# Innoptech/OpenFDCM

Hardware: AMD Instinct MI355X
Metric: template matches/sec (DT3 build + DefaultMatch/BatchOptimize search per frame) (higher is better)
Workload: dtype f32

## Files before the change

openfdcm_amd/csrc/fdcm_search.hip:

```cpp
#include <algorithm>
#include <cstdio>
#include <atomic>
#include <chrono>
#include <cstring>
#include <numeric>
#include <thread>

#include "fdcm_internal.h"
#include "fdcm_score.h"

namespace fdcm {

struct SearchParams {
    const float* vol;
    const float* keys;
    int W, H, m;
    float tx, ty;
    const float* tlines;
    const long long* toffsets;
    const float* tlengths;
    const int* tsorted;
    int T;
    const float* slines;
    const float* s_sorted_len;
    const int* s_sorted_idx;
    int n_s;
    int maxT, maxS, window;
    int optimizer;
    int batch;
    int win;
    int base;
    const long long* cand_offsets;
    const int2* pairs;
    int pairs_stride;
    int bpt;
    const int2* work;
    long long ncand;
    int nblocks;
    int lds_lines;
    const unsigned short* host_bins;
    fdcm_match* records;
    int* flags;
    int* evals;
    unsigned long long* counters;
};

static constexpr int kWavesPerBlock = 4;

struct OptState {
    VolRef V;
    const float* L;
    float* sc;
    int n_t, lane, B, WIN;
    bool batch_rule;
    bool reset_back;
    unsigned H;
    float tx, ty, savx, savy;
    int lim_p, lim_n;
};

template <bool BUF32>
__device__ __forceinline__ void score_range(const OptState& o, int dir, int k_from, int cnt, int dst, bool with_zero) {
    const int h = o.lane >> 5, slot = o.lane & 31;
    const int total = cnt + (with_zero ? 1 : 0);
    for (int s0 = 0; s0 < total; s0 += 32) {
        const int idx = s0 + slot - (with_zero ? 1 : 0);
        const bool act = idx < cnt;
        const int k = idx < 0 ? 0 : k_from + dir * idx;
        const float trx = idx < 0 ? 0.f : (float)k * o.savx, try_ = idx < 0 ? 0.f : (float)k * o.savy;
        const float s = pair_score<BUF32>(o.V, o.L, o.n_t, o.tx + trx, o.ty + try_, o.H, h, act);
        if (act && h == 0) o.sc[idx < 0 ? 2 * o.WIN : dst + idx] = s;
    }
}

template <bool BUF32>
__device__ __forceinline__ void optimise(const OptState& o, float& best, int& best_k, int& n_eval) {
    const int WIN = o.WIN, B = o.B;
    const int h = o.lane >> 5, slot = o.lane & 31;
    const int have_p = min(WIN, o.lim_p >= 1 ? o.lim_p : 0);
    const int have_n = min(WIN, o.lim_n <= -1 ? -o.lim_n : 0);
    if (1 + have_p + have_n <= 32) {
        const int idx = slot - 1;
        const bool is_p = idx >= 0 && idx < have_p, is_n = idx >= have_p && idx < have_p + have_n;
        const bool act = slot == 0 || is_p || is_n;
        const int k = is_p ? 1 + idx : (is_n ? -1 - (idx - have_p) : 0);
        const float trx = slot == 0 ? 0.f : (float)k * o.savx, try_ = slot == 0 ? 0.f : (float)k * o.savy;
        const float s = pair_score<BUF32>(o.V, o.L, o.n_t, o.tx + trx, o.ty + try_, o.H, h, act);
        if (act && h == 0) o.sc[slot == 0 ? 2 * WIN : (is_p ? idx : WIN + (idx - have_p))] = s;
    } else {
        score_range<BUF32>(o, +1, 1, have_p, 0, true);
        score_range<BUF32>(o, -1, -1, have_n, WIN, false);
    }
    const float init = o.sc[2 * WIN];
    n_eval += 1;
    best = init;
    float back = init;
    for (int dir = 1; dir >= -1; dir -= 2) {
        if (dir < 0 && o.reset_back) back = init;
        const int lim = dir > 0 ? o.lim_p : o.lim_n;
        const int off = dir > 0 ? 0 : WIN;
        int win0 = dir;
        int have = dir > 0 ? have_p : have_n;
        for (int k0 = dir; dir > 0 ? k0 <= lim : k0 >= lim; k0 += dir * B) {
            int nb = dir > 0 ? (lim - k0 + 1) : (k0 - lim + 1);
            if (nb > B) nb = B;
            float bmin = 0.f, blast = 0.f;
            int bmin_k = 0;
            for (int c0 = 0; c0 < nb;) {
                int rel = dir > 0 ? (k0 + c0 - win0) : (win0 - (k0 - c0));
                if (rel >= have) {
                    win0 = k0 + dir * c0;
                    const int left = dir > 0 ? (lim - win0 + 1) : (win0 - lim + 1);
                    have = min(WIN, left);
                    score_range<BUF32>(o, dir, win0, have, off, false);
                    rel = 0;
                }
                const int take = min(nb - c0, have - rel);
                for (int e0 = 0; e0 < take; e0 += 64) {
                    const int n = min(64, take - e0);
                    const float s = o.lane < n ? o.sc[off + rel + e0 + o.lane] : f_inf();
                    const bool is_nan = s != s;
                    const unsigned long long nans = __ballot(is_nan);
                    const float mn = wave_min_f(is_nan ? f_inf() : s);
                    const unsigned long long at = __ballot(o.lane < n && !is_nan && s == mn);
                    if (c0 == 0 && e0 == 0 && (nans & 1ull)) {
                        bmin = f_nan(); bmin_k = k0;
                    } else if (at != 0 && ((c0 == 0 && e0 == 0) || mn < bmin)) {
                        bmin = mn; bmin_k = k0 + dir * (c0 + e0 + __ffsll((long long)at) - 1);
                    }
                    blast = __shfl(s, n - 1);
                }
                c0 += take;
            }
            n_eval += nb;
            if (bmin > back) break;
            back = bmin;
            if (bmin < best) { best = bmin; best_k = bmin_k; }
            if (o.batch_rule && bmin < blast) break;
        }
    }
}

__global__ void k_pairs(const SearchParams P) {
    const int gidx = blockIdx.x * blockDim.x + threadIdx.x;
    const int per = P.maxT;
    if (gidx >= P.T * per) return;
    const int t = gidx / per, j = gidx - t * per;
    const long long l0 = P.toffsets[t];
    const int n_t = (int)(P.toffsets[t + 1] - l0);
    int2* out = const_cast<int2*>(P.pairs) + (size_t)t * P.pairs_stride + (size_t)j * P.window;
    if (j >= n_t) {
        for (int wi = 0; wi < P.window; ++wi) out[wi] = make_int2(-1, -1);
        return;
    }
    const int tl_local = P.tsorted[l0 + j];
    const float tlen = P.tlengths[l0 + tl_local];
    const int centre = binary_search_greater(P.s_sorted_len, P.n_s, tlen);
    int rb, re;
    centered_range(centre, P.n_s, P.maxS, rb, re);
    for (int wi = 0; wi < P.window; ++wi) out[wi] = make_int2(tl_local, P.s_sorted_idx[rb + wi]);
}

static constexpr int kWorkBins = 8192;
__device__ __forceinline__ int work_key(int scene_idx) { return scene_idx & (kWorkBins - 1); }
__device__ __forceinline__ int work_rank(int* bins, int key, bool valid, int lane) {
    (void)lane;
    return valid ? atomicAdd(&bins[key], 1) : 0;
}
__device__ __forceinline__ void work_scan(int* bins, int* partial, int tid) {
    constexpr int PER = kWorkBins / 1024;
    int loc[PER], sum = 0;
#pragma unroll
    for (int q = 0; q < PER; ++q) { loc[q] = sum; sum += bins[tid * PER + q]; }
    partial[tid] = sum;
    __syncthreads();
    for (int d = 1; d < 1024; d <<= 1) {
        const int v = tid >= d ? partial[tid - d] : 0;
        __syncthreads();
        partial[tid] += v;
        __syncthreads();
    }
    const int excl = partial[tid] - sum;
#pragma unroll
    for (int q = 0; q < PER; ++q) bins[tid * PER + q] = excl + loc[q];
}

__global__ void __launch_bounds__(1024) k_worklist(const SearchParams P, long long n_slots, int2* __restrict__ work) {
    __shared__ int bins[kWorkBins];
    __shared__ int partial[1024];
    const int tid = threadIdx.x, lane = tid & 63;
    for (int i = tid; i < kWorkBins; i += 1024) bins[i] = 0;
    {
        constexpr int RR = 16;
        int2 pr[RR];
        int rk[RR];
#pragma unroll
        for (int r = 0; r < RR; ++r) {
            const long long i = (long long)r * 1024 + tid;
            pr[r] = i < n_slots ? P.pairs[i] : make_int2(-1, -1);
        }
        __syncthreads();
#pragma unroll
        for (int r = 0; r < RR; ++r) rk[r] = work_rank(bins, work_key(pr[r].y), pr[r].x >= 0, lane);
        __syncthreads();
        work_scan(bins, partial, tid);
        __syncthreads();
#pragma unroll
        for (int r = 0; r < RR; ++r) {
            if (pr[r].x < 0) continue;
            const long long i = (long long)r * 1024 + tid;
            const int t = (int)(i / P.pairs_stride);
            work[bins[work_key(pr[r].y)] + rk[r]] = make_int2(t, (int)(i - (long long)t * P.pairs_stride));
        }
    }
}

static constexpr int kWlSlotsPerBlock = 16 * 1024;
__global__ void __launch_bounds__(1024) k_wl_count(const SearchParams P, long long n_slots, int* __restrict__ ghist) {
    __shared__ int bins[kWorkBins];
    const int tid = threadIdx.x;
    for (int i = tid; i < kWorkBins; i += 1024) bins[i] = 0;
    __syncthreads();
    const long long b0 = (long long)blockIdx.x * kWlSlotsPerBlock;
#pragma unroll
    for (int r = 0; r < 16; ++r) {
        const long long i = b0 + (long long)r * 1024 + tid;
        const int2 pr = i < n_slots ? P.pairs[i] : make_int2(-1, -1);
        if (pr.x >= 0) atomicAdd(&bins[work_key(pr.y)], 1);
    }
    __syncthreads();
    for (int i = tid; i < kWorkBins; i += 1024)
        if (bins[i]) atomicAdd(&ghist[i], bins[i]);
}
__global__ void __launch_bounds__(1024) k_wl_starts(int* __restrict__ ghist, int* __restrict__ cursor) {
    __shared__ int bins[kWorkBins];
    __shared__ int partial[1024];
    const int tid = threadIdx.x;
    for (int i = tid; i < kWorkBins; i += 1024) { bins[i] = ghist[i]; cursor[i] = 0; }
    __syncthreads();
    work_scan(bins, partial, tid);
    __syncthreads();
    for (int i = tid; i < kWorkBins; i += 1024) ghist[i] = bins[i];
}
__global__ void __launch_bounds__(1024) k_wl_scatter(const SearchParams P, long long n_slots, const int* __restrict__ starts,
                                                     int* __restrict__ cursor, int2* __restrict__ work) {
    __shared__ int bins[kWorkBins];
    const int tid = threadIdx.x, lane = tid & 63;
    for (int i = tid; i < kWorkBins; i += 1024) bins[i] = 0;
    __syncthreads();
    const long long b0 = (long long)blockIdx.x * kWlSlotsPerBlock;
    int2 pr[16];
    int rk[16];
#pragma unroll
    for (int r = 0; r < 16; ++r) {
        const long long i = b0 + (long long)r * 1024 + tid;
        pr[r] = i < n_slots ? P.pairs[i] : make_int2(-1, -1);
    }
#pragma unroll
    for (int r = 0; r < 16; ++r) rk[r] = work_rank(bins, work_key(pr[r].y), pr[r].x >= 0, lane);
    __syncthreads();
    for (int i = tid; i < kWorkBins; i += 1024) {
        const int c = bins[i];
        bins[i] = c ? starts[i] + atomicAdd(&cursor[i], c) : 0;
    }
    __syncthreads();
#pragma unroll
    for (int r = 0; r < 16; ++r) {
        if (pr[r].x < 0) continue;
        const long long i = b0 + (long long)r * 1024 + tid;
        const int t = (int)(i / P.pairs_stride);
        work[bins[work_key(pr[r].y)] + rk[r]] = make_int2(t, (int)(i - (long long)t * P.pairs_stride));
    }
}

static constexpr int kSearchWavesPerEU = 4;
template <bool BUF32>
__global__ void __launch_bounds__(64 * kWavesPerBlock, kSearchWavesPerEU) k_search(const SearchParams P) {
    extern __shared__ float lds[];
    const int tid = threadIdx.x, lane = tid & 63, wave = tid >> 6;
    int t, local;
    if (P.work) {
        const long long w = (long long)blockIdx.x * kWavesPerBlock + wave;
        if (w >= P.ncand) return;
        const int2 e = P.work[w >> 1];
        t = e.x;
        local = e.y * 2 + (int)(w & 1);
    } else {
        t = blockIdx.x / P.bpt;
        local = (blockIdx.x - t * P.bpt) * kWavesPerBlock + wave;
    }
    const long long l0 = P.toffsets[t];
    const int n_t = (int)(P.toffsets[t + 1] - l0);
    const int count_t = 2 * min(n_t, P.maxT) * P.window;
    if (local >= count_t) return;
    float* s_keys = lds + (size_t)wave * (P.m + 5 * P.lds_lines + 2 * P.win + 1);
    float* L = s_keys + P.m;
    float* sc = L + 5 * P.lds_lines;
    for (int i = lane; i < P.m; i += 64) s_keys[i] = P.keys[i];
    const long long cand = P.cand_offsets[t] + local;
    const VolRef V = make_volref(P.vol, ivol_slice_floats(P.W, P.H), P.m, BUF32);

    const int flip = local & 1, pair = local >> 1;
    const int2 pr = P.pairs[(size_t)t * P.pairs_stride + pair];
    const int tl_local = pr.x, scene_idx = pr.y;
    float tl[4], sl[4];
#pragma unroll
    for (int c = 0; c < 4; ++c) { tl[c] = P.tlines[(l0 + tl_local) * 4 + c]; sl[c] = P.slines[(size_t)scene_idx * 4 + c]; }
    const float* s_tl = P.tlines + l0 * 4;
    float T1[6], T2[6], T[6];
    align_pair(tl, sl, T1, T2);
#pragma unroll
    for (int c = 0; c < 6; ++c) T[c] = flip ? T2[c] : T1[c];
    float mnx = f_inf(), mny = f_inf(), mxx = -f_inf(), mxy = -f_inf();
    for (int i = lane; i < n_t; i += 64) {
        const float* p = s_tl + 4 * i;
        const float x1 = (T[0] * p[0] + T[1] * p[1]) + T[2], y1 = (T[3] * p[0] + T[4] * p[1]) + T[5];
        const float x2 = (T[0] * p[2] + T[1] * p[3]) + T[2], y2 = (T[3] * p[2] + T[4] * p[3]) + T[5];
        int bin;
        if (P.host_bins) {
            bin = (int)P.host_bins[(size_t)cand * P.lds_lines + i];
        } else {
            const float angle = atanf_glibc((y2 - y1) / (x2 - x1));
            bin = closest_orientation(s_keys, P.m, angle);
        }
        float* d = L + 5 * i;
        d[0] = x1; d[1] = y1; d[2] = x2; d[3] = y2; d[4] = line_slice_word(V, bin);
        mnx = std_min(mnx, std_min(x1, x2)); mxx = std_max(mxx, std_max(x1, x2));
        mny = std_min(mny, std_min(y1, y2)); mxy = std_max(mxy, std_max(y1, y2));
    }
    mnx = wave_min_f(mnx); mny = wave_min_f(mny); mxx = wave_max_f(mxx); mxy = wave_max_f(mxy);

    bool valid = true;
    float ax = sl[2] - sl[0], ay = sl[3] - sl[1];
    {
        const float nrm = sqrtf(ax * ax + ay * ay);
        ax = ax / nrm; ay = ay / nrm;
    }
    if (relatively_equal(f_abs(ax) + f_abs(ay), 0.f)) valid = false;
    float savx = 0.f, savy = 0.f, min_mul = 0.f, max_mul = 0.f;
    if (valid) {
        rasterize_vector(ax, ay, savx, savy);
        minmax_translation(mnx, mny, mxx, mxy, savx, savy, (float)P.W, (float)P.H, P.tx, P.ty, min_mul, max_mul);
        if (!f_isfinite(min_mul) || !f_isfinite(max_mul)) valid = false;
    }
    float best = 0.f;
    int best_k = 0, n_eval = 0;
    if (valid) {
        OptState o;
        o.V = V; o.L = L; o.sc = sc; o.n_t = n_t; o.H = (unsigned)P.H; o.tx = P.tx; o.ty = P.ty;
        o.savx = savx; o.savy = savy; o.lane = lane;
        o.B = P.optimizer == FDCM_BATCH_OPTIMIZE ? P.batch : 1; o.WIN = P.win; o.batch_rule = P.optimizer == FDCM_BATCH_OPTIMIZE;
        o.reset_back = P.optimizer == FDCM_INDULGENT_OPTIMIZE;
        const long long lp = (long long)max_mul, ln = (long long)min_mul;
        o.lim_p = (int)std::min<long long>(std::max<long long>(lp, -(1ll << 30)), 1ll << 30);
        o.lim_n = (int)std::min<long long>(std::max<long long>(ln, -(1ll << 30)), 1ll << 30);
        optimise<BUF32>(o, best, best_k, n_eval);
    }
    if (lane == 0) {
        fdcm_match r;
        r.tmpl_idx = P.base + t;
        r.score = best;
        const float trx = best_k == 0 ? 0.f : (float)best_k * savx, try_ = best_k == 0 ? 0.f : (float)best_k * savy;
        r.transform[0] = T[0]; r.transform[1] = T[1]; r.transform[2] = T[2] + trx;
        r.transform[3] = T[3]; r.transform[4] = T[4]; r.transform[5] = T[5] + try_;
        if (valid) P.records[cand] = r;
        P.flags[cand] = valid ? 1 : 0;
        P.evals[cand] = (int)n_eval;
    }
}

static constexpr int kChunk = 1024;
__global__ void __launch_bounds__(256) k_chunk_counts(const int* __restrict__ flags, const int* __restrict__ evals,
                                                      long long n, int* __restrict__ counts, int* __restrict__ evsums) {
    __shared__ int part[4], epart[4];
    const long long c0 = (long long)blockIdx.x * kChunk;
    int s = 0, e = 0;
    for (int i = threadIdx.x; i < kChunk; i += 256) {
        if (c0 + i < n) { s += flags[c0 + i]; e += evals[c0 + i]; }
    }
    for (int d = 32; d >= 1; d >>= 1) { s += __shfl_xor(s, d); e += __shfl_xor(e, d); }
    if ((threadIdx.x & 63) == 0) { part[threadIdx.x >> 6] = s; epart[threadIdx.x >> 6] = e; }
    __syncthreads();
    if (threadIdx.x == 0) {
        counts[blockIdx.x] = part[0] + part[1] + part[2] + part[3];
        evsums[blockIdx.x] = epart[0] + epart[1] + epart[2] + epart[3];
    }
}
__global__ void __launch_bounds__(1024) k_scatter(const fdcm_match* __restrict__ records, const int* __restrict__ flags,
                                                  long long n, const int* __restrict__ counts,
                                                  const int* __restrict__ evsums, int nchunks,
                                                  fdcm_match* __restrict__ out, unsigned long long* __restrict__ counters,
                                                  fdcm_match* __restrict__ out2, unsigned long long* __restrict__ counters2) {
    __shared__ long long wsum[16];
    __shared__ long long chunk_base;
    const int tid = threadIdx.x, lane = tid & 63, wave = tid >> 6;
    long long s = 0;
    for (int i = tid; i < (int)blockIdx.x; i += 1024) s += counts[i];
    for (int d = 32; d >= 1; d >>= 1) s += __shfl_xor(s, d);
    if (lane == 0) wsum[wave] = s;
    __syncthreads();
    if (tid == 0) {
        long long b = 0;
        for (int w = 0; w < 16; ++w) b += wsum[w];
        chunk_base = b;
    }
    __syncthreads();
    const long long i = (long long)blockIdx.x * kChunk + tid;
    const int f = i < n ? flags[i] : 0;
    int incl = f;
    for (int d = 1; d < 64; d <<= 1) {
        const int o = __shfl_up(incl, d);
        if (lane >= d) incl += o;
    }
    __syncthreads();
    if (lane == 63) wsum[wave] = incl;
    __syncthreads();
    long long wbase = 0;
    for (int w = 0; w < wave; ++w) wbase += wsum[w];
    if (f) {
        const fdcm_match r = records[i];
        out[chunk_base + wbase + incl - 1] = r;
        if (out2) out2[chunk_base + wbase + incl - 1] = r;
    }
    if ((int)blockIdx.x == nchunks - 1) {
        if (tid == 1023) {
            counters[2] = (unsigned long long)(chunk_base + wbase + incl);
            if (counters2) counters2[2] = (unsigned long long)(chunk_base + wbase + incl);
        }
        long long ev = 0;
        for (int i2 = tid; i2 < nchunks; i2 += 1024) ev += evsums[i2];
        for (int d = 32; d >= 1; d >>= 1) ev += __shfl_xor(ev, d);
        __syncthreads();
        if (lane == 0) wsum[wave] = ev;
        __syncthreads();
        if (tid == 0) {
            long long tot = 0;
            for (int w = 0; w < 16; ++w) tot += wsum[w];
            counters[0] = (unsigned long long)tot;
            if (counters2) counters2[0] = (unsigned long long)tot;
        }
    }
}

static constexpr int kCompactChunks = 64;
__global__ void __launch_bounds__(1024) k_compact(const fdcm_match* __restrict__ records, const int* __restrict__ flags,
                                                  const int* __restrict__ evals, long long n, int nchunks,
                                                  fdcm_match* __restrict__ out, unsigned long long* __restrict__ counters,
                                                  fdcm_match* __restrict__ out2, unsigned long long* __restrict__ counters2) {
    __shared__ long long wsum[16];
    __shared__ long long chunk_base;
    const int tid = threadIdx.x, lane = tid & 63, wave = tid >> 6;
    const long long i = (long long)blockIdx.x * kChunk + tid;
    const int f = i < n ? flags[i] : 0;
    fdcm_match r{};
    if (f) r = records[i];
    long long s = 0;
    {
        const int4* f4 = reinterpret_cast<const int4*>(flags);
        const long long n4 = (long long)blockIdx.x * (kChunk / 4);
        for (long long q = tid; q < n4; q += 1024) { const int4 v = f4[q]; s += v.x + v.y + v.z + v.w; }
    }
    for (int d = 32; d >= 1; d >>= 1) s += __shfl_xor(s, d);
    if (lane == 0) wsum[wave] = s;
    __syncthreads();
    if (tid == 0) {
        long long b = 0;
        for (int w = 0; w < 16; ++w) b += wsum[w];
        chunk_base = b;
    }
    int incl = f;
    for (int d = 1; d < 64; d <<= 1) {
        const int o = __shfl_up(incl, d);
        if (lane >= d) incl += o;
    }
    __syncthreads();
    const long long cb = chunk_base;
    __syncthreads();
    if (lane == 63) wsum[wave] = incl;
    __syncthreads();
    long long wbase = 0;
    for (int w = 0; w < wave; ++w) wbase += wsum[w];
    if (f) {
        out[cb + wbase + incl - 1] = r;
        if (out2) out2[cb + wbase + incl - 1] = r;
    }
    if ((int)blockIdx.x == nchunks - 1) {
        if (tid == 1023) {
            counters[2] = (unsigned long long)(cb + wbase + incl);
            if (counters2) counters2[2] = (unsigned long long)(cb + wbase + incl);
        }
        long long ev = 0;
        for (long long i2 = tid; i2 < n; i2 += 1024) ev += evals[i2];
        for (int d = 32; d >= 1; d >>= 1) ev += __shfl_xor(ev, d);
        __syncthreads();
        if (lane == 0) wsum[wave] = ev;
        __syncthreads();
        if (tid == 0) {
            long long tot = 0;
            for (int w = 0; w < 16; ++w) tot += wsum[w];
            counters[0] = (unsigned long long)tot;
            if (counters2) counters2[0] = (unsigned long long)tot;
        }
    }
}

struct SearchLayout {
    int64_t maxT = 0, maxS = 0;
    std::vector<long long> coff;
    int64_t cpt_max = 0, ncand = 0, pairs_stride = 0;
    int nchunks = 0;
    size_t o_lines = 0, o_len = 0, o_idx = 0, o_coff = 0, scene = 0;
    size_t records = 0, flags = 0, counters = 64, pairs = 0, work_list = 0, work = 0, bins = 0, out = 0;
};
static SearchLayout search_layout(const fdcm_templates* t, int64_t n_scene, int64_t maxT, int64_t maxS) {
    SearchLayout L;
    L.maxT = std::min<int64_t>(std::max<int64_t>(maxT, 0), std::max<int64_t>(t->max_lines, 0));
    L.maxS = std::min<int64_t>(std::max<int64_t>(maxS, 0), n_scene);
    L.coff.assign((size_t)t->T + 1, 0);
    for (int64_t i = 0; i < t->T; ++i) {
        const int64_t nt = t->offsets[i + 1] - t->offsets[i];
        const int64_t c = 2 * std::min<int64_t>(nt, L.maxT) * L.maxS;
        L.coff[i + 1] = L.coff[i] + c;
        L.cpt_max = std::max(L.cpt_max, c);
    }
    L.ncand = L.coff[t->T];
    L.nchunks = (int)((L.ncand + kChunk - 1) / kChunk);
    L.pairs_stride = L.maxT * L.maxS;
    auto align16 = [](size_t v) { return (v + 15) & ~(size_t)15; };
    const size_t n_s = (size_t)n_scene, ncand = (size_t)L.ncand;
    L.o_len = align16(n_s * 16), L.o_idx = L.o_len + align16(n_s * 4), L.o_coff = L.o_idx + align16(n_s * 4);
    L.scene = L.o_coff + align16(L.coff.size() * 8);
    L.records = ncand * sizeof(fdcm_match);
    L.flags = 2 * (ncand + (size_t)L.nchunks) * sizeof(int);
    L.pairs = std::max<size_t>(16, (size_t)t->T * (size_t)L.pairs_stride * sizeof(int2));
    L.work_list = align16(ncand / 2 * sizeof(int2));
    L.work = L.work_list + 2 * (size_t)kWorkBins * sizeof(int);
    L.bins = ncand * (size_t)std::max<int64_t>(1, t->max_lines) * sizeof(unsigned short);
    L.out = (ncand + 1) * sizeof(fdcm_match);
    return L;
}

int64_t search_capacity(const fdcm_templates* t, int64_t n_scene, int64_t maxT, int64_t maxS) {
    return search_layout(t, n_scene, maxT, maxS).ncand;
}

bool orientation_bins_on_host() {
    static const bool on_host = [] {
        const bool forced = test_switches().host_bins;
        const bool differs = fdcm_selftest_atanf(0, 65537, (1ull << 32) / 65537) != 0;
        if (forced || differs)
            fprintf(stderr, "libfdcm_hip: orientation bins of the candidates come from this machine's libm on host threads (%s); "
                            "searches are slower than with the device's atanf (fdcm_orientation_bins_mode() == 1)\n",
                    differs ? "its atanf differs from the glibc 2.35 restatement the device runs" : "FDCM_FORCE_HOST_BINS is set");
        return forced || differs;
    }();
    return on_host;
}

static void reserve_workspaces(fdcm_featuremap* fm, const SearchLayout& L, bool host_bins) {
    fm->search.stage.reserve(L.scene); fm->search.scene.reserve(L.scene);
    fm->search.records.reserve(L.records); fm->search.flags.reserve(L.flags); fm->search.counter.reserve(L.counters);
    fm->search.pairs.reserve(L.pairs); fm->search.work.reserve(L.work);
    if (host_bins) { fm->search.bins_stage.reserve(L.bins); fm->search.bins.reserve(L.bins); }
}

void reserve_search(fdcm_featuremap* fm, const fdcm_templates* t, int64_t n_scene, int64_t maxT, int64_t maxS) {
    if (!t || t->T == 0 || n_scene <= 0) return;
    FDCM_HIP(hipSetDevice(fm->device));
    const SearchLayout L = search_layout(t, n_scene, maxT, maxS);
    if (L.ncand == 0) return;
    reserve_workspaces(fm, L, orientation_bins_on_host());
    fm->search.cnt.reserve(L.counters);
}

void run_search(fdcm_featuremap* fm, const fdcm_templates* t, const float* scene, int64_t n_scene, int64_t maxT,
                int64_t maxS, int optimizer, int64_t batch, int32_t base, fdcm_match* out_device, fdcm_match** out_host,
                int64_t* n_out) {
    *n_out = 0;
    fm->last_search = fdcm_search_timing{};
    if (t->T == 0 || n_scene == 0 || (fm->W == 0 && fm->H == 0)) return;
    const bool host_bins_needed = orientation_bins_on_host();
    FDCM_HIP(hipSetDevice(fm->device));
    ensure_stream(fm);
    hipStream_t st = fm->stream;
    const int n_s = (int)n_scene;
    const SearchLayout L = search_layout(t, n_scene, maxT, maxS);
    maxT = L.maxT; maxS = L.maxS;
    const int window = (int)maxS;
    std::vector<float> slen((size_t)n_s);
    for (int i = 0; i < n_s; ++i) {
        const float dx = scene[4 * i + 2] - scene[4 * i], dy = scene[4 * i + 3] - scene[4 * i + 1];
        slen[i] = std::sqrt(dx * dx + dy * dy);
    }
    std::vector<long> sidx((size_t)n_s);
    std::iota(sidx.begin(), sidx.end(), 0);
    std::sort(sidx.begin(), sidx.end(), [&slen](long const i1, long const i2) { return slen[i1] > slen[i2]; });
    const std::vector<long long>& coff = L.coff;
    const long long ncand = L.ncand;
    fm->last_search.candidates = ncand;
    if (ncand == 0) return;
    if (fm->holds != VolStage::integrated) throw std::string("the feature map holds a partial build (no line integral): nothing to search");
    const int64_t B = optimizer == FDCM_BATCH_OPTIMIZE ? std::max<int64_t>(1, batch) : 1;
    if (B > 4096) throw std::string("batch_size above 4096 is not supported");
    const int win = B <= 15 ? (int)((15 / B) * B) : (int)B;
    const int lds_lines = (int)std::max<int64_t>(1, t->max_lines);
    const size_t lds = (size_t)kWavesPerBlock * ((size_t)fm->m + 5 * (size_t)lds_lines + 2 * (size_t)win + 1) * sizeof(float);
    if (lds > 160 * 1024) throw std::string("scene/template too large for the search kernel's LDS staging");
    if (host_bins_needed && fm->m > 65535) throw std::string("host-side orientation bins need depth <= 65535");
    reserve_workspaces(fm, L, host_bins_needed);
    char* hs = (char*)fm->search.stage.p;
    std::memcpy(hs + L.o_lines, scene, (size_t)n_s * 16);
    float* hl = (float*)(hs + L.o_len);
    int* hi = (int*)(hs + L.o_idx);
    for (int i = 0; i < n_s; ++i) { hl[i] = slen[sidx[i]]; hi[i] = (int)sidx[i]; }
    std::memcpy(hs + L.o_coff, coff.data(), coff.size() * 8);
    hipStream_t sp = st;
    if (!fm->shares_gpu) {
        if (!fm->prep_stream) {
            FDCM_HIP(hipStreamCreateWithFlags(&fm->prep_stream, hipStreamNonBlocking));
            FDCM_HIP(hipEventCreateWithFlags(&fm->prep_done, hipEventDisableTiming));
        }
        sp = fm->prep_stream;
    }
    FDCM_HIP(hipMemcpyAsync(fm->search.scene.p, hs, L.scene, hipMemcpyHostToDevice, sp));
    const int nchunks = L.nchunks;
    SearchParams P{};
    P.vol = fm->vol.as<float>();
    P.keys = (const float*)((const char*)fm->build.plan.p + fm->off_keys);
    P.W = (int)fm->W; P.H = (int)fm->H; P.m = (int)fm->m; P.tx = fm->tx; P.ty = fm->ty;
    P.tlines = t->d_lines.as<float>();
    P.toffsets = t->d_offsets.as<long long>();
    P.tlengths = t->d_lengths.as<float>();
    P.tsorted = t->d_sorted.as<int>();
    P.T = (int)t->T;
    const char* ds = (const char*)fm->search.scene.p;
    P.slines = (const float*)(ds + L.o_lines);
    P.s_sorted_len = (const float*)(ds + L.o_len);
    P.s_sorted_idx = (const int*)(ds + L.o_idx);
    P.n_s = n_s;
    P.maxT = (int)maxT; P.maxS = (int)maxS; P.window = window;
    P.optimizer = optimizer;
    P.batch = (int)B;
    P.win = win;
    P.base = base;
    P.cand_offsets = (const long long*)(ds + L.o_coff);
    P.bpt = (int)((L.cpt_max + kWavesPerBlock - 1) / kWavesPerBlock);
    P.ncand = ncand;
    P.lds_lines = lds_lines;
    P.records = fm->search.records.as<fdcm_match>();
    P.flags = fm->search.flags.as<int>();
    P.evals = P.flags + ncand + nchunks;
    P.counters = fm->search.counter.as<unsigned long long>();
    P.pairs_stride = (int)L.pairs_stride;
    P.pairs = fm->search.pairs.as<int2>();
    const bool buf32 = !test_switches().search_flat && (size_t)fm->m * ivol_slice_floats(fm->W, fm->H) * sizeof(float) < ((size_t)1 << 32);
    if (lds > 64 * 1024)
        FDCM_HIP(hipFuncSetAttribute(buf32 ? (const void*)k_search<true> : (const void*)k_search<false>,
                                     hipFuncAttributeMaxDynamicSharedMemorySize, (int)lds));
    hipEvent_t* ev = fm->timing.ev;
    const bool timed = fm->want_stage_events != 0;
    if (timed) FDCM_HIP(hipEventRecord(ev[6], st));
    hipLaunchKernelGGL(k_pairs, dim3((unsigned)(((size_t)t->T * maxT + 255) / 256)), dim3(256), 0, sp, P);
    const long long n_slots = (long long)t->T * P.pairs_stride;
    if (n_slots <= 0x7fffffffll) {
        if (n_slots <= kWlSlotsPerBlock) {
            hipLaunchKernelGGL(k_worklist, dim3(1), dim3(1024), 0, sp, P, n_slots, fm->search.work.as<int2>());
        } else {
            int* ghist = (int*)((char*)fm->search.work.p + L.work_list);
            int* cursor = ghist + kWorkBins;
            const unsigned nb = (unsigned)((n_slots + kWlSlotsPerBlock - 1) / kWlSlotsPerBlock);
            FDCM_HIP(hipMemsetAsync(ghist, 0, (size_t)kWorkBins * sizeof(int), sp));
            hipLaunchKernelGGL(k_wl_count, dim3(nb), dim3(1024), 0, sp, P, n_slots, ghist);
            hipLaunchKernelGGL(k_wl_starts, dim3(1), dim3(1024), 0, sp, ghist, cursor);
            hipLaunchKernelGGL(k_wl_scatter, dim3(nb), dim3(1024), 0, sp, P, n_slots, ghist, cursor, fm->search.work.as<int2>());
        }
        P.work = fm->search.work.as<int2>();
        P.nblocks = (int)(((ncand + kWavesPerBlock - 1) / kWavesPerBlock + 7) / 8 * 8);
    } else {
        P.work = nullptr;
        P.nblocks = (int)((size_t)t->T * P.bpt);
    }
    if (sp != st) {
        FDCM_HIP(hipEventRecord(fm->prep_done, sp));
        FDCM_HIP(hipStreamWaitEvent(st, fm->prep_done, 0));
    }
    if (host_bins_needed) {
        const size_t stride = (size_t)P.lds_lines;
        unsigned short* hb = (unsigned short*)fm->search.bins_stage.p;
        const float* keys = fm->keys.data();
        const int mkeys = (int)fm->m;
        std::vector<float> sorted_len((size_t)n_s);
        for (int i = 0; i < n_s; ++i) sorted_len[i] = slen[sidx[i]];
        const unsigned nthreads = std::max(1u, std::min(16u, std::thread::hardware_concurrency()));
        std::vector<std::thread> th;
        std::atomic<int64_t> next{0};
        const fdcm_templates* tt = t;
        for (unsigned w = 0; w < nthreads; ++w)
            th.emplace_back([&, tt] {
                for (int64_t ti; (ti = next.fetch_add(1)) < tt->T;) {
                    const int64_t l0 = tt->offsets[ti];
                    const int n_t = (int)(tt->offsets[ti + 1] - l0);
                    const int jmax = (int)std::min<int64_t>(n_t, maxT);
                    for (int j = 0; j < jmax; ++j) {
                        const int tl_local = tt->sorted[(size_t)l0 + j];
                        const float tlen = tt->lengths[(size_t)l0 + tl_local];
                        const int centre = binary_search_greater(sorted_len.data(), n_s, tlen);
                        int rb, re;
                        centered_range(centre, n_s, (int)maxS, rb, re);
                        for (int wi = 0; wi < window; ++wi) {
                            const int scene_idx = (int)sidx[rb + wi];
                            float T1[6], T2[6];
                            align_pair(&tt->lines[(size_t)(l0 + tl_local) * 4], scene + (size_t)scene_idx * 4, T1, T2);
                            for (int flip = 0; flip < 2; ++flip) {
                                const float* T = flip ? T2 : T1;
                                const long long cand = coff[ti] + 2ll * (j * window + wi) + flip;
                                unsigned short* out = hb + (size_t)cand * stride;
                                for (int i = 0; i < n_t; ++i) {
                                    const float* p = &tt->lines[(size_t)(l0 + i) * 4];
                                    const float x1 = (T[0] * p[0] + T[1] * p[1]) + T[2], y1 = (T[3] * p[0] + T[4] * p[1]) + T[5];
                                    const float x2 = (T[0] * p[2] + T[1] * p[3]) + T[2], y2 = (T[3] * p[2] + T[4] * p[3]) + T[5];
                                    const float angle = std::atan((y2 - y1) / (x2 - x1));
                                    out[i] = (unsigned short)closest_orientation(keys, mkeys, angle);
                                }
                            }
                        }
                    }
                }
            });
        for (auto& x : th) x.join();
        FDCM_HIP(hipMemcpyAsync(fm->search.bins.p, hb, (size_t)ncand * stride * sizeof(unsigned short), hipMemcpyHostToDevice, st));
        P.host_bins = fm->search.bins.as<unsigned short>();
    }
    if (buf32) hipLaunchKernelGGL(k_search<true>, dim3((unsigned)P.nblocks), dim3(64 * kWavesPerBlock), lds, st, P);
    else hipLaunchKernelGGL(k_search<false>, dim3((unsigned)P.nblocks), dim3(64 * kWavesPerBlock), lds, st, P);
    fdcm_match* dst = out_device;
    if (!dst) {
        fm->search.out.reserve(L.out);
        dst = fm->search.out.as<fdcm_match>();
        P.counters = reinterpret_cast<unsigned long long*>(dst + ncand);
    }
    int* d_counts = P.flags + ncand;
    int* d_evsums = P.evals + ncand;
    fdcm_match* host_out = nullptr;
    unsigned long long* host_cnt = nullptr;
    if (out_host) {
        *out_host = result_acquire((size_t)(ncand + 1) * sizeof(fdcm_match));
        FDCM_HIP(hipHostGetDevicePointer((void**)&host_out, *out_host, 0));
        host_cnt = reinterpret_cast<unsigned long long*>(host_out + ncand);
    } else {
        fm->search.cnt.reserve(L.counters);
        FDCM_HIP(hipHostGetDevicePointer((void**)&host_cnt, fm->search.cnt.p, 0));
    }
    if (nchunks <= kCompactChunks && !test_switches().search_compact2) {
        hipLaunchKernelGGL(k_compact, dim3((unsigned)nchunks), dim3(1024), 0, st, P.records, P.flags, P.evals, ncand, nchunks, dst, P.counters,
                           host_out, host_cnt);
    } else {
        hipLaunchKernelGGL(k_chunk_counts, dim3((unsigned)nchunks), dim3(256), 0, st, P.flags, P.evals, ncand, d_counts, d_evsums);
        hipLaunchKernelGGL(k_scatter, dim3((unsigned)nchunks), dim3(1024), 0, st, P.records, P.flags, ncand, d_counts, d_evsums,
                           nchunks, dst, P.counters, host_out, host_cnt);
    }
    if (timed) FDCM_HIP(hipEventRecord(ev[7], st));
    FDCM_HIP(hipGetLastError());
    unsigned long long hc[3] = {0, 0, 0};
    FDCM_HIP(hipStreamSynchronize(st));
    finish_build(fm);
    std::memcpy(hc, out_host ? (const void*)(*out_host + ncand) : (const void*)fm->search.cnt.p, sizeof hc);
    *n_out = (int64_t)hc[2];
    fm->last_search.evaluations = (int64_t)hc[0];
    if (timed) FDCM_HIP(hipEventElapsedTime(&fm->last_search.kernel_ms, ev[6], ev[7]));
    fm->last_search.total_ms = fm->last_search.kernel_ms;
}

}
```

Before: 63.95 million.

## Process eight candidates per wave with shared LDS table and paired half-wave staging

Each wave now handles a group of eight candidates instead of one. Per-candidate setup (alignment transform, step vector, translation limits) is computed lane-parallel and kept in an LDS table. Templates with at most 32 lines get aligned two candidates at a time, one per half-wave. LDS line staging is sized for several candidates at once within a per-block budget. This amortizes setup and reduces idle lanes on short templates, at the cost of more LDS per wave, fewer blocks, and serialized optimisation within each wave.

```diff
diff --git a/openfdcm_amd/csrc/fdcm_search.hip b/openfdcm_amd/csrc/fdcm_search.hip
--- a/openfdcm_amd/csrc/fdcm_search.hip
+++ b/openfdcm_amd/csrc/fdcm_search.hip
@@ -34,6 +34,7 @@
     const int2* pairs;
     int pairs_stride;
     int bpt;
+    int areas;
     const int2* work;
     long long ncand;
     int nblocks;
@@ -46,6 +47,12 @@
 };
 
 static constexpr int kWavesPerBlock = 4;
+static constexpr int kGroup = 8;
+enum { F_T0 = 0, F_SAVX = 6, F_SAVY, F_T, F_LOCAL, F_NT, F_FLAGS, F_MNX, F_MNY, F_MXX, F_MXY, F_LIMP, F_LIMN, F_BEST, F_K, F_EVAL, kTabFields };
+enum { kPresent = 1, kValid = 2 };
+FDCM_HD size_t search_wave_floats(int m, int lds_lines, int areas, int win) {
+    return (size_t)m + (size_t)kTabFields * kGroup + (size_t)5 * lds_lines * areas + 2 * (size_t)win + 1;
+}
 
 struct OptState {
     VolRef V;
@@ -274,98 +281,209 @@
 }
 
 static constexpr int kSearchWavesPerEU = 4;
+
+__device__ __forceinline__ void aligned_line(const SearchParams& P, const VolRef& V, const float* s_keys, const float* s_tl,
+                                             const float* T, int i, long long cand, float* L, float& mnx, float& mny,
+                                             float& mxx, float& mxy) {
+    const float* p = s_tl + 4 * i;
+    const float x1 = (T[0] * p[0] + T[1] * p[1]) + T[2], y1 = (T[3] * p[0] + T[4] * p[1]) + T[5];
+    const float x2 = (T[0] * p[2] + T[1] * p[3]) + T[2], y2 = (T[3] * p[2] + T[4] * p[3]) + T[5];
+    int bin;
+    if (P.host_bins) {
+        bin = (int)P.host_bins[(size_t)cand * P.lds_lines + i];
+    } else {
+        const float angle = atanf_glibc((y2 - y1) / (x2 - x1));
+        bin = closest_orientation(s_keys, P.m, angle);
+    }
+    float* d = L + 5 * i;
+    d[0] = x1; d[1] = y1; d[2] = x2; d[3] = y2; d[4] = line_slice_word(V, bin);
+    mnx = std_min(mnx, std_min(x1, x2)); mxx = std_max(mxx, std_max(x1, x2));
+    mny = std_min(mny, std_min(y1, y2)); mxy = std_max(mxy, std_max(y1, y2));
+}
+__device__ __forceinline__ void wave_phase() {
+    __builtin_amdgcn_fence(__ATOMIC_ACQ_REL, "wavefront");
+    __builtin_amdgcn_wave_barrier();
+}
+__device__ __forceinline__ int uniform_i(int v) { return __builtin_amdgcn_readfirstlane(v); }
+__device__ __forceinline__ float uniform_f(float v) { return __int_as_float(__builtin_amdgcn_readfirstlane(__float_as_int(v))); }
+
 template <bool BUF32>
 __global__ void __launch_bounds__(64 * kWavesPerBlock, kSearchWavesPerEU) k_search(const SearchParams P) {
     extern __shared__ float lds[];
     const int tid = threadIdx.x, lane = tid & 63, wave = tid >> 6;
-    int t, local;
+    long long w0 = 0;
+    int t_tm = 0, lb_tm = 0;
     if (P.work) {
-        const long long w = (long long)blockIdx.x * kWavesPerBlock + wave;
-        if (w >= P.ncand) return;
-        const int2 e = P.work[w >> 1];
-        t = e.x;
-        local = e.y * 2 + (int)(w & 1);
+        w0 = ((long long)blockIdx.x * kWavesPerBlock + wave) * kGroup;
+        if (w0 >= P.ncand) return;
     } else {
-        t = blockIdx.x / P.bpt;
-        local = (blockIdx.x - t * P.bpt) * kWavesPerBlock + wave;
-    }
-    const long long l0 = P.toffsets[t];
-    const int n_t = (int)(P.toffsets[t + 1] - l0);
-    const int count_t = 2 * min(n_t, P.maxT) * P.window;
-    if (local >= count_t) return;
-    float* s_keys = lds + (size_t)wave * (P.m + 5 * P.lds_lines + 2 * P.win + 1);
-    float* L = s_keys + P.m;
-    float* sc = L + 5 * P.lds_lines;
+        t_tm = blockIdx.x / P.bpt;
+        lb_tm = ((blockIdx.x - t_tm * P.bpt) * kWavesPerBlock + wave) * kGroup;
+        const int n_tm = (int)(P.toffsets[t_tm + 1] - P.toffsets[t_tm]);
+        if (lb_tm >= 2 * min(n_tm, P.maxT) * P.window) return;
+    }
+    float* s_keys = lds + (size_t)wave * search_wave_floats(P.m, P.lds_lines, P.areas, P.win);
+    float* tab = s_keys + P.m;
+    float* areas = tab + kTabFields * kGroup;
+    float* sc = areas + (size_t)5 * P.lds_lines * P.areas;
     for (int i = lane; i < P.m; i += 64) s_keys[i] = P.keys[i];
-    const long long cand = P.cand_offsets[t] + local;
     const VolRef V = make_volref(P.vol, ivol_slice_floats(P.W, P.H), P.m, BUF32);
 
-    const int flip = local & 1, pair = local >> 1;
-    const int2 pr = P.pairs[(size_t)t * P.pairs_stride + pair];
-    const int tl_local = pr.x, scene_idx = pr.y;
-    float tl[4], sl[4];
-#pragma unroll
-    for (int c = 0; c < 4; ++c) { tl[c] = P.tlines[(l0 + tl_local) * 4 + c]; sl[c] = P.slines[(size_t)scene_idx * 4 + c]; }
-    const float* s_tl = P.tlines + l0 * 4;
-    float T1[6], T2[6], T[6];
-    align_pair(tl, sl, T1, T2);
-#pragma unroll
-    for (int c = 0; c < 6; ++c) T[c] = flip ? T2[c] : T1[c];
-    float mnx = f_inf(), mny = f_inf(), mxx = -f_inf(), mxy = -f_inf();
-    for (int i = lane; i < n_t; i += 64) {
-        const float* p = s_tl + 4 * i;
-        const float x1 = (T[0] * p[0] + T[1] * p[1]) + T[2], y1 = (T[3] * p[0] + T[4] * p[1]) + T[5];
-        const float x2 = (T[0] * p[2] + T[1] * p[3]) + T[2], y2 = (T[3] * p[2] + T[4] * p[3]) + T[5];
-        int bin;
-        if (P.host_bins) {
-            bin = (int)P.host_bins[(size_t)cand * P.lds_lines + i];
+    if (lane < kGroup) {
+        int t, local;
+        bool present = true;
+        if (P.work) {
+            const long long w = w0 + lane;
+            present = w < P.ncand;
+            const int2 e = P.work[(present ? w : w0) >> 1];
+            t = e.x;
+            local = e.y * 2 + (int)(w & 1);
         } else {
-            const float angle = atanf_glibc((y2 - y1) / (x2 - x1));
-            bin = closest_orientation(s_keys, P.m, angle);
-        }
-        float* d = L + 5 * i;
-        d[0] = x1; d[1] = y1; d[2] = x2; d[3] = y2; d[4] = line_slice_word(V, bin);
-        mnx = std_min(mnx, std_min(x1, x2)); mxx = std_max(mxx, std_max(x1, x2));
-        mny = std_min(mny, std_min(y1, y2)); mxy = std_max(mxy, std_max(y1, y2));
-    }
-    mnx = wave_min_f(mnx); mny = wave_min_f(mny); mxx = wave_max_f(mxx); mxy = wave_max_f(mxy);
-
-    bool valid = true;
-    float ax = sl[2] - sl[0], ay = sl[3] - sl[1];
-    {
-        const float nrm = sqrtf(ax * ax + ay * ay);
-        ax = ax / nrm; ay = ay / nrm;
-    }
-    if (relatively_equal(f_abs(ax) + f_abs(ay), 0.f)) valid = false;
-    float savx = 0.f, savy = 0.f, min_mul = 0.f, max_mul = 0.f;
-    if (valid) {
-        rasterize_vector(ax, ay, savx, savy);
-        minmax_translation(mnx, mny, mxx, mxy, savx, savy, (float)P.W, (float)P.H, P.tx, P.ty, min_mul, max_mul);
-        if (!f_isfinite(min_mul) || !f_isfinite(max_mul)) valid = false;
-    }
-    float best = 0.f;
-    int best_k = 0, n_eval = 0;
-    if (valid) {
-        OptState o;
-        o.V = V; o.L = L; o.sc = sc; o.n_t = n_t; o.H = (unsigned)P.H; o.tx = P.tx; o.ty = P.ty;
-        o.savx = savx; o.savy = savy; o.lane = lane;
-        o.B = P.optimizer == FDCM_BATCH_OPTIMIZE ? P.batch : 1; o.WIN = P.win; o.batch_rule = P.optimizer == FDCM_BATCH_OPTIMIZE;
-        o.reset_back = P.optimizer == FDCM_INDULGENT_OPTIMIZE;
-        const long long lp = (long long)max_mul, ln = (long long)min_mul;
-        o.lim_p = (int)std::min<long long>(std::max<long long>(lp, -(1ll << 30)), 1ll << 30);
-        o.lim_n = (int)std::min<long long>(std::max<long long>(ln, -(1ll << 30)), 1ll << 30);
-        optimise<BUF32>(o, best, best_k, n_eval);
-    }
-    if (lane == 0) {
-        fdcm_match r;
-        r.tmpl_idx = P.base + t;
-        r.score = best;
-        const float trx = best_k == 0 ? 0.f : (float)best_k * savx, try_ = best_k == 0 ? 0.f : (float)best_k * savy;
-        r.transform[0] = T[0]; r.transform[1] = T[1]; r.transform[2] = T[2] + trx;
-        r.transform[3] = T[3]; r.transform[4] = T[4]; r.transform[5] = T[5] + try_;
-        if (valid) P.records[cand] = r;
-        P.flags[cand] = valid ? 1 : 0;
-        P.evals[cand] = (int)n_eval;
+            t = t_tm;
+            local = lb_tm + lane;
+        }
+        const long long l0 = P.toffsets[t];
+        const int n_t = (int)(P.toffsets[t + 1] - l0);
+        if (local >= 2 * min(n_t, P.maxT) * P.window) present = false;
+        float T[6] = {0.f, 0.f, 0.f, 0.f, 0.f, 0.f};
+        float savx = 0.f, savy = 0.f;
+        bool valid = false;
+        if (present) {
+            const int flip = local & 1, pair = local >> 1;
+            const int2 pr = P.pairs[(size_t)t * P.pairs_stride + pair];
+            const int tl_local = pr.x, scene_idx = pr.y;
+            float tl[4], sl[4];
+#pragma unroll
+            for (int c = 0; c < 4; ++c) { tl[c] = P.tlines[(l0 + tl_local) * 4 + c]; sl[c] = P.slines[(size_t)scene_idx * 4 + c]; }
+            float T1[6], T2[6];
+            align_pair(tl, sl, T1, T2);
+#pragma unroll
+            for (int c = 0; c < 6; ++c) T[c] = flip ? T2[c] : T1[c];
+            float ax = sl[2] - sl[0], ay = sl[3] - sl[1];
+            const float nrm = sqrtf(ax * ax + ay * ay);
+            ax = ax / nrm; ay = ay / nrm;
+            valid = !relatively_equal(f_abs(ax) + f_abs(ay), 0.f);
+            if (valid) rasterize_vector(ax, ay, savx, savy);
+        }
+#pragma unroll
+        for (int c = 0; c < 6; ++c) tab[(F_T0 + c) * kGroup + lane] = T[c];
+        tab[F_SAVX * kGroup + lane] = savx;
+        tab[F_SAVY * kGroup + lane] = savy;
+        tab[F_T * kGroup + lane] = __int_as_float(t);
+        tab[F_LOCAL * kGroup + lane] = __int_as_float(local);
+        tab[F_NT * kGroup + lane] = __int_as_float(n_t);
+        tab[F_FLAGS * kGroup + lane] = __int_as_float((present ? kPresent : 0) | (valid ? kValid : 0));
+    }
+    wave_phase();
+
+    for (int s0 = 0; s0 < kGroup; s0 += P.areas) {
+        const int s1 = min(kGroup, s0 + P.areas);
+        for (int c = s0; c < s1;) {
+            if (!(uniform_i(__float_as_int(tab[F_FLAGS * kGroup + c])) & kPresent)) break;
+            const int t = uniform_i(__float_as_int(tab[F_T * kGroup + c]));
+            const int n_t = uniform_i(__float_as_int(tab[F_NT * kGroup + c]));
+            const float* s_tl = P.tlines + P.toffsets[t] * 4;
+            const long long cand0 = P.cand_offsets[t];
+            float mnx = f_inf(), mny = f_inf(), mxx = -f_inf(), mxy = -f_inf();
+            if (n_t <= 32 && !(c & 1) && c + 1 < s1) {
+                const int i = lane & 31, cc = c + (lane >> 5);
+                float T[6];
+#pragma unroll
+                for (int q = 0; q < 6; ++q) T[q] = tab[(F_T0 + q) * kGroup + cc];
+                const bool present = (__float_as_int(tab[F_FLAGS * kGroup + cc]) & kPresent) != 0;
+                if (i < n_t && present)
+                    aligned_line(P, V, s_keys, s_tl, T, i, cand0 + __float_as_int(tab[F_LOCAL * kGroup + cc]),
+                                 areas + (size_t)5 * P.lds_lines * (cc - s0), mnx, mny, mxx, mxy);
+                for (int d = 16; d >= 1; d >>= 1) {
+                    mnx = std_min(mnx, __shfl_xor(mnx, d)); mny = std_min(mny, __shfl_xor(mny, d));
+                    mxx = std_max(mxx, __shfl_xor(mxx, d)); mxy = std_max(mxy, __shfl_xor(mxy, d));
+                }
+                if (i == 0) {
+                    tab[F_MNX * kGroup + cc] = mnx; tab[F_MNY * kGroup + cc] = mny;
+                    tab[F_MXX * kGroup + cc] = mxx; tab[F_MXY * kGroup + cc] = mxy;
+                }
+                c += 2;
+            } else {
+                float T[6];
+#pragma unroll
+                for (int q = 0; q < 6; ++q) T[q] = uniform_f(tab[(F_T0 + q) * kGroup + c]);
+                const long long cand = cand0 + uniform_i(__float_as_int(tab[F_LOCAL * kGroup + c]));
+                float* L = areas + (size_t)5 * P.lds_lines * (c - s0);
+                for (int i = lane; i < n_t; i += 64) aligned_line(P, V, s_keys, s_tl, T, i, cand, L, mnx, mny, mxx, mxy);
+                mnx = wave_min_f(mnx); mny = wave_min_f(mny); mxx = wave_max_f(mxx); mxy = wave_max_f(mxy);
+                if (lane == 0) {
+                    tab[F_MNX * kGroup + c] = mnx; tab[F_MNY * kGroup + c] = mny;
+                    tab[F_MXX * kGroup + c] = mxx; tab[F_MXY * kGroup + c] = mxy;
+                }
+                c += 1;
+            }
+        }
+        wave_phase();
+        if (lane >= s0 && lane < s1) {
+            const int fl = __float_as_int(tab[F_FLAGS * kGroup + lane]);
+            if ((fl & (kPresent | kValid)) == (kPresent | kValid)) {
+                float min_mul = 0.f, max_mul = 0.f;
+                minmax_translation(tab[F_MNX * kGroup + lane], tab[F_MNY * kGroup + lane], tab[F_MXX * kGroup + lane],
+                                   tab[F_MXY * kGroup + lane], tab[F_SAVX * kGroup + lane], tab[F_SAVY * kGroup + lane],
+                                   (float)P.W, (float)P.H, P.tx, P.ty, min_mul, max_mul);
+                if (!f_isfinite(min_mul) || !f_isfinite(max_mul)) {
+                    tab[F_FLAGS * kGroup + lane] = __int_as_float(fl & ~kValid);
+                } else {
+                    const long long lp = (long long)max_mul, ln = (long long)min_mul;
+                    tab[F_LIMP * kGroup + lane] = __int_as_float((int)std::min<long long>(std::max<long long>(lp, -(1ll << 30)), 1ll << 30));
+                    tab[F_LIMN * kGroup + lane] = __int_as_float((int)std::min<long long>(std::max<long long>(ln, -(1ll << 30)), 1ll << 30));
+                }
+            }
+        }
+        wave_phase();
+        for (int c = s0; c < s1; ++c) {
+            const int fl = uniform_i(__float_as_int(tab[F_FLAGS * kGroup + c]));
+            if (!(fl & kPresent)) break;
+            float best = 0.f;
+            int best_k = 0, n_eval = 0;
+            if (fl & kValid) {
+                OptState o;
+                o.V = V; o.L = areas + (size_t)5 * P.lds_lines * (c - s0); o.sc = sc;
+                o.n_t = uniform_i(__float_as_int(tab[F_NT * kGroup + c]));
+                o.H = (unsigned)P.H; o.tx = P.tx; o.ty = P.ty;
+                o.savx = uniform_f(tab[F_SAVX * kGroup + c]); o.savy = uniform_f(tab[F_SAVY * kGroup + c]); o.lane = lane;
+                o.B = P.optimizer == FDCM_BATCH_OPTIMIZE ? P.batch : 1; o.WIN = P.win; o.batch_rule = P.optimizer == FDCM_BATCH_OPTIMIZE;
+                o.reset_back = P.optimizer == FDCM_INDULGENT_OPTIMIZE;
+                o.lim_p = uniform_i(__float_as_int(tab[F_LIMP * kGroup + c]));
+                o.lim_n = uniform_i(__float_as_int(tab[F_LIMN * kGroup + c]));
+                optimise<BUF32>(o, best, best_k, n_eval);
+            }
+            if (lane == 0) {
+                tab[F_BEST * kGroup + c] = best;
+                tab[F_K * kGroup + c] = __int_as_float(best_k);
+                tab[F_EVAL * kGroup + c] = __int_as_float(n_eval);
+            }
+        }
+        wave_phase();
+    }
+
+    if (lane < kGroup) {
+        const int fl = __float_as_int(tab[F_FLAGS * kGroup + lane]);
+        if (fl & kPresent) {
+            const int t = __float_as_int(tab[F_T * kGroup + lane]);
+            const long long cand = P.cand_offsets[t] + __float_as_int(tab[F_LOCAL * kGroup + lane]);
+            const bool valid = (fl & kValid) != 0;
+            if (valid) {
+                const float savx = tab[F_SAVX * kGroup + lane], savy = tab[F_SAVY * kGroup + lane];
+                const int r_k = __float_as_int(tab[F_K * kGroup + lane]);
+                fdcm_match r;
+                r.tmpl_idx = P.base + t;
+                r.score = tab[F_BEST * kGroup + lane];
+                const float trx = r_k == 0 ? 0.f : (float)r_k * savx, try_ = r_k == 0 ? 0.f : (float)r_k * savy;
+                r.transform[0] = tab[F_T0 * kGroup + lane]; r.transform[1] = tab[(F_T0 + 1) * kGroup + lane];
+                r.transform[2] = tab[(F_T0 + 2) * kGroup + lane] + trx;
+                r.transform[3] = tab[(F_T0 + 3) * kGroup + lane]; r.transform[4] = tab[(F_T0 + 4) * kGroup + lane];
+                r.transform[5] = tab[(F_T0 + 5) * kGroup + lane] + try_;
+                P.records[cand] = r;
+            }
+            P.flags[cand] = valid ? 1 : 0;
+            P.evals[cand] = __float_as_int(tab[F_EVAL * kGroup + lane]);
+        }
     }
 }
 
@@ -509,6 +627,16 @@
     std::vector<long long> coff;
     int64_t cpt_max = 0, ncand = 0, pairs_stride = 0;
     int nchunks = 0;
+    int lds_lines = 1;
+    static constexpr size_t kLdsPerCU = 160 * 1024;
+    size_t lds_bytes(int m, int win, int areas) const {
+        return (size_t)kWavesPerBlock * search_wave_floats(m, lds_lines, areas, win) * sizeof(float);
+    }
+    int areas(int m, int win) const {
+        int a = kGroup;
+        while (a > 1 && lds_bytes(m, win, a) > kLdsPerCU / 4) a >>= 1;
+        return a;
+    }
     size_t o_lines = 0, o_len = 0, o_idx = 0, o_coff = 0, scene = 0;
     size_t records = 0, flags = 0, counters = 64, pairs = 0, work_list = 0, work = 0, bins = 0, out = 0;
 };
@@ -526,6 +654,7 @@
     L.ncand = L.coff[t->T];
     L.nchunks = (int)((L.ncand + kChunk - 1) / kChunk);
     L.pairs_stride = L.maxT * L.maxS;
+    L.lds_lines = (int)std::max<int64_t>(1, t->max_lines);
     auto align16 = [](size_t v) { return (v + 15) & ~(size_t)15; };
     const size_t n_s = (size_t)n_scene, ncand = (size_t)L.ncand;
     L.o_len = align16(n_s * 16), L.o_idx = L.o_len + align16(n_s * 4), L.o_coff = L.o_idx + align16(n_s * 4);
@@ -603,9 +732,9 @@
     const int64_t B = optimizer == FDCM_BATCH_OPTIMIZE ? std::max<int64_t>(1, batch) : 1;
     if (B > 4096) throw std::string("batch_size above 4096 is not supported");
     const int win = B <= 15 ? (int)((15 / B) * B) : (int)B;
-    const int lds_lines = (int)std::max<int64_t>(1, t->max_lines);
-    const size_t lds = (size_t)kWavesPerBlock * ((size_t)fm->m + 5 * (size_t)lds_lines + 2 * (size_t)win + 1) * sizeof(float);
-    if (lds > 160 * 1024) throw std::string("scene/template too large for the search kernel's LDS staging");
+    const int areas = L.areas((int)fm->m, win);
+    const size_t lds = L.lds_bytes((int)fm->m, win, areas);
+    if (lds > SearchLayout::kLdsPerCU) throw std::string("scene/template too large for the search kernel's LDS staging");
     if (host_bins_needed && fm->m > 65535) throw std::string("host-side orientation bins need depth <= 65535");
     reserve_workspaces(fm, L, host_bins_needed);
     char* hs = (char*)fm->search.stage.p;
@@ -644,9 +773,10 @@
     P.win = win;
     P.base = base;
     P.cand_offsets = (const long long*)(ds + L.o_coff);
-    P.bpt = (int)((L.cpt_max + kWavesPerBlock - 1) / kWavesPerBlock);
+    P.bpt = (int)((L.cpt_max + kWavesPerBlock * kGroup - 1) / (kWavesPerBlock * kGroup));
+    P.areas = areas;
     P.ncand = ncand;
-    P.lds_lines = lds_lines;
+    P.lds_lines = L.lds_lines;
     P.records = fm->search.records.as<fdcm_match>();
     P.flags = fm->search.flags.as<int>();
     P.evals = P.flags + ncand + nchunks;
@@ -675,7 +805,7 @@
             hipLaunchKernelGGL(k_wl_scatter, dim3(nb), dim3(1024), 0, sp, P, n_slots, ghist, cursor, fm->search.work.as<int2>());
         }
         P.work = fm->search.work.as<int2>();
-        P.nblocks = (int)(((ncand + kWavesPerBlock - 1) / kWavesPerBlock + 7) / 8 * 8);
+        P.nblocks = (int)(((ncand + kWavesPerBlock * kGroup - 1) / (kWavesPerBlock * kGroup) + 7) / 8 * 8);
     } else {
         P.work = nullptr;
         P.nblocks = (int)((size_t)t->T * P.bpt);
```

After: 55.14 million. -13.8%, worse.
